# mlrun/mlrun

Hardware: NVIDIA H100
Metric: events/sec (higher is better)
Workload: dtype f32 in / f64 accumulate

## Files before the change

mlrun_b200/csrc/b2s_rowthread.cuh:

```cuda
#pragma once
#include <cuda.h>
#include <type_traits>

#include "b2s_device.cuh"
#include "b2s_hash.cuh"

namespace b2s {

constexpr int kRTMaxCatCols = 16;
constexpr int kRTCatsInline = 4;
constexpr int kRTMaxCats = 256;

template <int NCH, int NS>
struct RTParams {
  const char* rows;
  int64_t row_stride;
  int64_t n_rows;
  float* out;
  int32_t* status;
  int32_t n_in, out_cols, n_models, vote_kind, out_is_int, fast_epilogue, tile_rows, pitch, stages, vec_ok;
  int32_t n_cat_cols, n_cat;
  int32_t one_sync;
  int32_t use_bulk;
  float* peers[8];
  int64_t peer_off;
  int32_t n_peers;
  MergeSig sig;
  const double* wcat;
  const double* vote_w_g;
  const ModelDesc* models;
  const int32_t* classes;
  double w[NCH * 4][NS];
  float fill[NCH * 4];
  float lim[NCH * 4];
  double bias[NS];
  double vote_w[NS];
  int32_t cat_col[kRTMaxCatCols];
  int32_t cat_off[kRTMaxCatCols];
  int32_t cat_sw[kRTMaxCatCols];
  int32_t cat_base[kRTMaxCatCols];
  int32_t cat_cnt[kRTMaxCatCols];
  float cat_fill[kRTMaxCatCols];
  float cat_inl[kRTMaxCatCols][kRTCatsInline];
  int32_t cat_first[kRTMaxCatCols];
  int32_t cat_dense[kRTMaxCatCols];
  float cat_val[kRTMaxCats];
  struct CatFast {
    int32_t off_b;
    int32_t sw_b;
    int32_t first;
    int32_t cnt;
    int32_t woff_b;
    float fill;
    int32_t pad[2];
  };
  CatFast catf[kRTMaxCatCols];
  int32_t cats_fast;
  int32_t zero_woff_b;
  int32_t dead_tail;
  int32_t pad_fast;
  const long long* g_keys;
  const TableSlot* g_slots;
  uint64_t g_mask;
  const float* g_values;
  long long g_missing_row;
};

struct RowPadded {
  const float* xr;
  __device__ __forceinline__ float4 chunk(int ch) const { return *reinterpret_cast<const float4*>(xr + ch * 4); }
  __device__ __forceinline__ float at2(int off, int) const { return xr[off]; }
  __device__ __forceinline__ float at_b(int off_b, int) const { return *reinterpret_cast<const float*>(reinterpret_cast<const char*>(xr) + off_b); }
};
struct RowSwizzled {
  const float* box0;
  int box_words;
  int r7s;
  __device__ __forceinline__ float4 chunk(int ch) const {
    return *reinterpret_cast<const float4*>(box0 + (ch >> 3) * box_words + (((ch & 7) << 2) ^ r7s));
  }
  __device__ __forceinline__ float at2(int off, int sw) const { return box0[off + (sw ^ r7s)]; }
  __device__ __forceinline__ float at_b(int off_b, int sw_b) const {
    return *reinterpret_cast<const float*>(reinterpret_cast<const char*>(box0) + off_b + (sw_b ^ (r7s << 2)));
  }
};

template <int NCH, int NS, int CH0, int CH1, typename Row>
__device__ __forceinline__ void rt_slice(const RTParams<NCH, NS>& p, const Row (&xr)[1], double (&acc)[1][NS]) {
  constexpr int RPT = 1;
  constexpr int BATCH = 4;
#pragma unroll
  for (int b = CH0; b < CH1; b += BATCH) {
    double xd[RPT][BATCH * 4];
#pragma unroll
    for (int cb = 0; cb < BATCH; ++cb) {
      const int ch = b + cb;
      if (ch < CH1) {
#pragma unroll
        for (int i = 0; i < RPT; ++i) {
          const float4 v = xr[i].chunk(ch);
          const float xs[4] = {v.x, v.y, v.z, v.w};
#pragma unroll
          for (int u = 0; u < 4; ++u) {
            const int c = ch * 4 + u;
            float x = xs[u];
            x = !(fabsf(x) <= p.lim[c]) ? p.fill[c] : x;
            xd[i][cb * 4 + u] = (double)x;
          }
        }
      }
    }
#pragma unroll
    for (int cb = 0; cb < BATCH; ++cb) {
      const int ch = b + cb;
      if (ch < CH1) {
#pragma unroll
        for (int u = 0; u < 4; ++u) {
          const int c = ch * 4 + u;
#pragma unroll
          for (int k = 0; k < NS; ++k)
#pragma unroll
            for (int i = 0; i < RPT; ++i) acc[i][k] = fma(p.w[c][k], xd[i][cb * 4 + u], acc[i][k]);
        }
      }
    }
  }
}

template <int NCH, int NS>
__device__ __noinline__ int rt_cat_search(const RTParams<NCH, NS>& p, int cc, float x) {
  const int b0 = p.cat_base[cc], cnt = p.cat_cnt[cc];
  int j = p.n_cat;
  if (cnt <= kRTCatsInline) {
#pragma unroll
    for (int qq = kRTCatsInline - 1; qq >= 0; --qq) j = (x == p.cat_inl[cc][qq]) ? b0 + qq : j;
  } else {
    for (int qq = cnt - 1; qq >= 0; --qq) j = (x == p.cat_val[b0 + qq]) ? b0 + qq : j;
  }
  return j;
}

template <int NCH, int NS, int Q0, int TPR, typename Row>
__device__ __forceinline__ void rt_cats(const RTParams<NCH, NS>& p, const Row (&xr)[1], const double* __restrict__ s_wcat,
                                        double (&acc)[1][NS]) {
  constexpr int RPT = 1;
  constexpr int ITERS = (kRTMaxCatCols - Q0 + TPR - 1) / TPR;
  if (p.cats_fast) {
    const char* wb = reinterpret_cast<const char*>(s_wcat);
#pragma unroll
    for (int it = 0; it < ITERS; ++it) {
      const int cc = Q0 + it * TPR;
      if (cc >= p.n_cat_cols) break;
      const typename RTParams<NCH, NS>::CatFast cf = p.catf[cc];
#pragma unroll
      for (int i = 0; i < RPT; ++i) {
        float x = xr[i].at_b(cf.off_b, cf.sw_b);
        x = (x != x) ? cf.fill : x;
        const int v = __float2int_rz(x);
        const unsigned jj = (unsigned)(v - cf.first);
        const bool miss = ((float)v != x) | (jj >= (unsigned)cf.cnt);
        const int a = miss ? p.zero_woff_b : cf.woff_b + (int)jj * (NS * 8);
        if constexpr (NS % 2 == 0) {
#pragma unroll
          for (int k = 0; k < NS; k += 2) {
            const double2 w2 = *reinterpret_cast<const double2*>(wb + a + k * 8);
            acc[i][k] += w2.x;
            acc[i][k + 1] += w2.y;
          }
        } else {
          const double* wc = reinterpret_cast<const double*>(wb + a);
#pragma unroll
          for (int k = 0; k < NS; ++k) acc[i][k] += wc[k];
        }
      }
    }
    return;
  }
#pragma unroll
  for (int it = 0; it < ITERS; ++it) {
    const int cc = Q0 + it * TPR;
    if (cc >= p.n_cat_cols) break;
#pragma unroll
    for (int i = 0; i < RPT; ++i) {
      float x = xr[i].at2(p.cat_off[cc], p.cat_sw[cc]);
      x = (x != x) ? p.cat_fill[cc] : x;
      int j;
      if (p.cat_dense[cc]) {
        const int v = __float2int_rz(x);
        const unsigned jj = (unsigned)(v - p.cat_first[cc]);
        j = ((float)v == x && jj < (unsigned)p.cat_cnt[cc]) ? p.cat_base[cc] + (int)jj : p.n_cat;
      } else {
        j = rt_cat_search(p, cc, x);
      }
      const double* wc = s_wcat + (size_t)j * NS;
#pragma unroll
      for (int k = 0; k < NS; ++k) acc[i][k] += wc[k];
    }
  }
}

template <int NCH, int NS, int TPR, int LIVE, typename Row>
__device__ __forceinline__ void rt_row_slices(const RTParams<NCH, NS>& p, int q, const Row (&xr)[1], const double* __restrict__ s_wcat,
                                              double (&acc)[1][NS]) {
  static_assert(LIVE % TPR == 0, "live chunks must split evenly over the row's threads");
  constexpr int CPT = LIVE / TPR;
  if (TPR == 1 || q == 0) {
    rt_slice<NCH, NS, 0, CPT>(p, xr, acc);
    rt_cats<NCH, NS, 0, TPR>(p, xr, s_wcat, acc);
  } else if (q == 1) {
    rt_slice<NCH, NS, (TPR > 1 ? CPT : 0), (TPR > 1 ? 2 * CPT : 0)>(p, xr, acc);
    rt_cats<NCH, NS, (TPR > 1 ? 1 : 0), TPR>(p, xr, s_wcat, acc);
  } else if (q == 2) {
    rt_slice<NCH, NS, (TPR > 2 ? 2 * CPT : 0), (TPR > 2 ? 3 * CPT : 0)>(p, xr, acc);
    rt_cats<NCH, NS, (TPR > 2 ? 2 : 0), TPR>(p, xr, s_wcat, acc);
  } else {
    rt_slice<NCH, NS, (TPR > 3 ? 3 * CPT : 0), (TPR > 3 ? 4 * CPT : 0)>(p, xr, acc);
    rt_cats<NCH, NS, (TPR > 3 ? 3 : 0), TPR>(p, xr, s_wcat, acc);
  }
}

__device__ __forceinline__ void mbar_init(uint64_t* bar, int count) {
  asm volatile("mbarrier.init.shared::cta.b64 [%0], %1;" ::"r"((uint32_t)__cvta_generic_to_shared(bar)), "r"(count));
}
__device__ __forceinline__ void mbar_expect_tx(uint64_t* bar, uint32_t bytes) {
  asm volatile("mbarrier.arrive.expect_tx.shared::cta.b64 _, [%0], %1;" ::"r"((uint32_t)__cvta_generic_to_shared(bar)), "r"(bytes)
               : "memory");
}
__device__ __forceinline__ void mbar_wait(uint64_t* bar, uint32_t parity) {
  const uint32_t a = (uint32_t)__cvta_generic_to_shared(bar);
  asm volatile(
      "{\n"
      ".reg .pred p;\n"
      "WAIT_%=:\n"
      "mbarrier.try_wait.parity.shared::cta.b64 p, [%0], %1;\n"
      "@p bra DONE_%=;\n"
      "bra WAIT_%=;\n"
      "DONE_%=:\n"
      "}\n" ::"r"(a), "r"(parity)
      : "memory");
}
__device__ __forceinline__ void bulk_load(void* smem_dst, const void* gsrc, uint32_t bytes, uint64_t* bar) {
  asm volatile("cp.async.bulk.shared::cluster.global.mbarrier::complete_tx::bytes [%0], [%1], %2, [%3];" ::"r"(
                   (uint32_t)__cvta_generic_to_shared(smem_dst)),
               "l"(gsrc), "r"(bytes), "r"((uint32_t)__cvta_generic_to_shared(bar))
               : "memory");
}

__device__ __forceinline__ void tensor_load_2d(void* smem_dst, const CUtensorMap* tmap, int x, int y, uint64_t* bar) {
  asm volatile(
      "cp.async.bulk.tensor.2d.shared::cluster.global.tile.mbarrier::complete_tx::bytes [%0], [%1, {%2, %3}], [%4];" ::"r"(
          (uint32_t)__cvta_generic_to_shared(smem_dst)),
// ... 1 lines not shown
      : "memory");
}

template <int NCH, int NS>
__device__ __noinline__ void rt_generic_epilogue(const RTParams<NCH, NS>& p, const double* sl, int64_t row, uint32_t st) {
  double pred[kMaxModels];
  for (int m = 0; m < p.n_models; ++m) {
    const ModelDesc md = p.models[m];
    pred[m] = apply_link(md, sl + md.score_off, p.classes);
  }
  KParams kp;
  kp.out = p.out;
  kp.out_cols = p.out_cols;
  kp.n_models = p.n_models;
  kp.vote_kind = p.vote_kind;
  kp.out_is_int = p.out_is_int;
  kp.vote_w = p.vote_w_g;
  kp.status = p.status;
  kp.n_peers = p.n_peers;
  kp.peer_off = p.peer_off;
  for (int g = 0; g < p.n_peers; ++g) kp.peers[g] = p.peers[g];
  vote_and_store(kp, pred, row, st);
}

template <int NCH, int NS, int TPR, int LM>
__global__ void __launch_bounds__(128 * TPR, TPR >= 4 ? 2 : (TPR == 2 ? 3 : 4))
    rowthread_kernel(const __grid_constant__ RTParams<NCH, NS> p, const __grid_constant__ CUtensorMap tmap) {
  constexpr int RPT = 1;
  static_assert(NCH % TPR == 0, "chunks must split evenly over the row's threads");
  constexpr int CPT = NCH / TPR;
  extern __shared__ __align__(16) unsigned char smem[];
  uint64_t* s_bar = reinterpret_cast<uint64_t*>(smem);
  double* s_wcat = reinterpret_cast<double*>(smem + 64);
  const size_t wcat_bytes = 64 + (((size_t)(p.n_cat + 1) * NS * 8 + 15) / 16) * 16;
  const bool one_sync = (LM == 2) && TPR > 1 && p.one_sync;
  constexpr size_t part_words = (size_t)(TPR - 1) * 128 * NS;
  double* s_part = reinterpret_cast<double*>(smem + wcat_bytes);
  float* s_tiles = reinterpret_cast<float*>(smem + wcat_bytes + (one_sync ? 2 : 1) * part_words * 8);
  if (LM == 2) {
    const uint32_t a = (uint32_t)__cvta_generic_to_shared(s_tiles);
    s_tiles += ((1024u - (a & 1023u)) & 1023u) >> 2;
  }

  const int tid = threadIdx.x;
  const int TR = p.tile_rows;
  const int S = p.stages;
  const int tile_words = (LM == 2) ? TR * NCH * 4 : TR * p.pitch;
  const int64_t n_tiles = (p.n_rows + TR - 1) / TR;
  const int TRT = TR / RPT;
  const int q = tid / TRT;
  const int r = tid - q * TRT;

  const int cprv = p.vec_ok ? (p.n_in >> 2) : p.n_in;
  const int r0 = tid / cprv, c0 = tid - r0 * cprv;
  const int dr = (int)blockDim.x / cprv, dc = (int)blockDim.x - dr * cprv;
  auto issue = [&](float* tile, int64_t row0) {
    int64_t left = p.n_rows - row0;
    const int rows = left < TR ? (left < 0 ? 0 : (int)left) : TR;
    const char* base = p.rows + row0 * p.row_stride;
    int rr = r0, cc = c0;
    if (p.vec_ok) {
      while (rr < rows) {
        cp_async16(tile + rr * p.pitch + cc * 4, base + (int64_t)rr * p.row_stride + cc * 16);
        rr += dr;
        cc += dc;
        if (cc >= cprv) {
          cc -= cprv;
          ++rr;
// ... 66 lines not shown
            unknown_bits = (unknown_bits & ~(1u << st)) | ((hit < 0 ? 1u : 0u) << st);
            bulk_load(s_tiles + st * tile_words + tid * p.pitch,
                      reinterpret_cast<const char*>(p.g_values + (hit < 0 ? p.g_missing_row : hit) * p.n_in), row_bytes, &s_bar[st]);
          }
          gk_cur = gk_nxt;
          g_probe_start(gk_cur);
          gk_nxt = g_key(g_tile_nxt);
          g_tile_nxt += gridDim.x;
        }
      } else if (tid < rows) {
        bulk_load(s_tiles + st * tile_words + tid * p.pitch, p.rows + (row0 + tid) * p.row_stride, row_bytes, &s_bar[st]);
      }
    }
  };
  if (bulk) {
    if (tid == 0) {
      for (int s = 0; s < S; ++s) mbar_init(&s_bar[s], 1);
      asm volatile("fence.mbarrier_init.release.cluster;" ::: "memory");
    }
    __syncthreads();
  }
  for (int s = 0; s < (one_sync ? S : S - 1); ++s) {
    const int64_t t = (int64_t)blockIdx.x + (int64_t)s * gridDim.x;
    if (bulk) {
      issue_bulk(s, t * TR);
    } else {
      if (t < n_tiles) issue(s_tiles + s * tile_words, t * TR);
      cp_async_commit();
    }
  }
  uint32_t phase_bits = 0;
  for (int i = tid; i < p.n_cat * NS; i += blockDim.x) s_wcat[i] = p.wcat[i];
  for (int i = tid; i < NS; i += blockDim.x) s_wcat[p.n_cat * NS + i] = 0.0;
  if (one_sync) __syncthreads();

  int stage = 0;
  uint32_t iter = 0;
  for (int64_t t = blockIdx.x; t < n_tiles; t += gridDim.x) {
    if (bulk) {
      mbar_wait(&s_bar[stage], (phase_bits >> stage) & 1u);
      phase_bits ^= (1u << stage);
    } else if (S == 2) cp_async_wait<0>();
    else if (S == 3) cp_async_wait<1>();
    else cp_async_wait<2>();
    if (!one_sync) {
      __syncthreads();
      const int64_t tn = t + (int64_t)(S - 1) * gridDim.x;
      int sn = stage + S - 1;
      if (sn >= S) sn -= S;
      if (bulk) {
        issue_bulk(sn, tn * TR);
      } else {
        if (tn < n_tiles) issue(s_tiles + sn * tile_words, tn * TR);
        cp_async_commit();
      }
    }
    const float* tile = s_tiles + stage * tile_words;
    const int64_t row0 = t * TR;
    const int live_rows = (int)(p.n_rows - row0 < (int64_t)TR ? p.n_rows - row0 : (int64_t)TR);
    const bool any_live = r < live_rows;
    using Row = typename std::conditional<LM == 2, RowSwizzled, RowPadded>::type;
    Row xr[RPT];
#pragma unroll
    for (int i = 0; i < RPT; ++i) {
      const int ri = r + i * TRT;
      if constexpr (LM == 2) {
        xr[i].box0 = tile + ri * 32;
        xr[i].box_words = TR * 32;
        xr[i].r7s = (r & 7) << 2;
      } else {
        xr[i].xr = tile + ri * p.pitch;
      }
    }
    double acc[RPT][NS];
#pragma unroll
    for (int i = 0; i < RPT; ++i)
#pragma unroll
      for (int k = 0; k < NS; ++k) acc[i][k] = 0.0;
    if (any_live) {
      if constexpr (LM == 2 && RPT == 1 && NCH >= 8 && (TPR == 1 || TPR == 2)) {
        if (p.dead_tail >= 4) rt_row_slices<NCH, NS, TPR, NCH - 4>(p, q, xr, s_wcat, acc);
        else if (p.dead_tail >= 2) rt_row_slices<NCH, NS, TPR, NCH - 2>(p, q, xr, s_wcat, acc);
        else rt_row_slices<NCH, NS, TPR, NCH>(p, q, xr, s_wcat, acc);
      } else {
        rt_row_slices<NCH, NS, TPR, NCH>(p, q, xr, s_wcat, acc);
      }
    }
    if (TPR > 1) {
      double* s_part_cur = s_part + (one_sync ? (size_t)(iter & 1) * part_words : 0);
      if (q > 0) {
#pragma unroll
        for (int i = 0; i < RPT; ++i) {
          double* part = s_part_cur + ((size_t)(q - 1) * 128 + r + i * TRT) * NS;
#pragma unroll
          for (int k = 0; k < NS; ++k) part[k] = acc[i][k];
        }
      }
      __syncthreads();
      if (one_sync) issue_bulk(stage, (t + (int64_t)S * gridDim.x) * TR);
      if (q == 0) {
#pragma unroll
        for (int i = 0; i < RPT; ++i)
#pragma unroll
          for (int qq = 1; qq < TPR; ++qq) {
            const double* o = s_part_cur + ((size_t)(qq - 1) * 128 + r + i * TRT) * NS;
#pragma unroll
            for (int k = 0; k < NS; ++k) acc[i][k] += o[k];
          }
      }
    }
#pragma unroll
    for (int i = 0; i < RPT; ++i) {
      const int64_t row = row0 + (r + i * TRT);
      if (q == 0 && r + i * TRT < live_rows) {
        uint32_t st = 0;
#pragma unroll
        for (int k = 0; k < NS; ++k) {
          acc[i][k] += p.bias[k];
          st |= (fabs(acc[i][k]) <= 1.7976931348623157e308) ? 0u : 1u;
        }
        if (LM == 1) st |= ((unknown_bits >> stage) & 1u) << 2;
        if (p.fast_epilogue) {
          if (p.vote_kind == 1) {
            double s = 0.0;
#pragma unroll
            for (int k = 0; k < NS; ++k) s = __dadd_rn(s, __dmul_rn(acc[i][k], p.vote_w[k]));
            store_word(p, row, 0, __float_as_uint((float)s));
          } else {
#pragma unroll
            for (int k = 0; k < NS; ++k)
              if (k < p.n_models) store_word(p, row, k, __float_as_uint((float)acc[i][k]));
          }
          if (p.status) p.status[row] = (int32_t)st;
        } else {
          double sl[NS];
#pragma unroll
          for (int k = 0; k < NS; ++k) sl[k] = acc[i][k];
          rt_generic_epilogue(p, sl, row, st);
        }
      }
    }
    ++stage;
    ++iter;
    if (stage == S) stage = 0;
  }
  cp_async_wait<0>();
  merge_signal(p.sig);
}

}
```

mlrun_b200/csrc/b2s_runtime.cu:

```cuda
#include <cuda_runtime.h>

#include <exception>

#include <algorithm>
#include <atomic>
#include <chrono>
#include <cmath>
#include <condition_variable>
#include <cstdarg>
#include <cstdio>
#include <cstdlib>
#include <cstring>
#include <deque>
#include <limits>
#include <map>
#include <memory>
#include <mutex>
#include <string>
#include <thread>
#include <vector>

#include "../../include/b200serve.h"
#include "b2s_internal.h"
#include "b2s_device.cuh"
// ... 128 lines not shown
  int fused_lag = -1;
  uint32_t fused_epoch = 0;
  size_t bytes = 0;
  bool connected = false;
  size_t buf_bytes() const { return (size_t)world * max_rows * out_cols * 4; }
  char* buf(int r, uint32_t e) const { return peer_base[r] + kCommHeader + (size_t)(e & (kCommSlots - 1u)) * buf_bytes(); }
  uint32_t* flags(int r) const { return reinterpret_cast<uint32_t*>(peer_base[r]); }
  uint32_t* counter() const { return reinterpret_cast<uint32_t*>(base.get()) + 64; }
  uint32_t* timeout_flag() const { return reinterpret_cast<uint32_t*>(base.get()) + 65; }
};

struct b2s_plan_s {
  int32_t n_in = 0;
  bool finalized = false;
  std::vector<float> fill;
  std::vector<std::vector<MapEntry>> maps;
  std::vector<int32_t> out_src, out_kind;
  std::vector<float> out_arg;
  std::vector<HostModel> models;
  int vote_kind = B2S_VOTE_NONE;
  std::vector<double> vote_w;
  int mode = MODE_STORE;
  int NS = 1;
  int out_cols = 0;
  int out_is_int = 0;
  KParams kp{};
  DeviceArray<char> d_blob;
  size_t blob_bytes = 0;
  int grid = 0, block = 0;
  int kernels_per_batch = 1;
  bool rt_ok = false;
  int rt_cat_cols = 0;
  int rt_NCH = 0, rt_NS = 0, rt_grid = 0, rt_smem = 0, rt_pitch = 0;
  std::vector<char> rt_blob;
  std::vector<void*> peers;
  int64_t peer_off = 0;
  struct b2s_comm_s* comm = nullptr;
  bool dense_ok = false;
  DenseParams dense{};
  int dense_smem = 0, dense_grid = 0;
  std::atomic<int32_t> last_kernel{B2S_KERNEL_NONE};
  bool t3_ok = false, t3_miss = false, t3_cat = false;
  bool any_cat = false;
  int t3_D = 0, t3_grid = 0, t3_block = 0, t3_smem = 0, t3_cols = 0, t3_parts = 0;
  T3Params t3{};
  T3Prep t3_prep{};
  int t3_prep_smem = 0;
  DeviceArray<char> d_t3_blob;
  const int32_t* d_t3_col_score = nullptr;
  const int32_t* d_t3_col_order = nullptr;
  const int32_t* d_t3_model_cols = nullptr;
  struct TreeScratch {
    DeviceArray<double> partial;
    DeviceArray<int32_t> row_bad;
    DeviceArray<uint32_t> xt;
    int64_t rows = 0;
    std::mutex mu;
    int reserve(int64_t n, int cols, int xt_words) {
      if (n <= rows) return B2S_OK;
      rows = 0;
      const int64_t cap = std::max<int64_t>((n + 63) / 64 * 64, 65536);
      if (int rc = allocate(partial, (size_t)cap * cols * 8)) return rc;
      if (int rc = allocate(row_bad, (size_t)cap * 4)) return rc;
      if (int rc = allocate(xt, (size_t)(cap / kT3TR) * xt_words * 4)) return rc;
      rows = cap;
      return B2S_OK;
// ... 82 lines not shown
    if (cudaGetDriverEntryPoint("cuTensorMapEncodeTiled", &sym, cudaEnableDefault, &q) != cudaSuccess || q != cudaDriverEntryPointSuccess) {
      cudaGetLastError();
      sym = nullptr;
    }
    return reinterpret_cast<EncodeTiledFn>(sym);
  }();
  return fn;
}
static bool encode_rows_map(CUtensorMap* map, const void* rows, int64_t n_rows, int64_t stride, int n_in, int tile_rows) {
  EncodeTiledFn enc = tensor_map_encoder();
  if (!enc) return false;
  cuuint64_t gdim[2] = {(cuuint64_t)n_in, (cuuint64_t)n_rows};
  cuuint64_t gstride[1] = {(cuuint64_t)stride};
  cuuint32_t box[2] = {32u, (cuuint32_t)tile_rows};
  cuuint32_t estr[2] = {1u, 1u};
  return enc(map, CU_TENSOR_MAP_DATA_TYPE_FLOAT32, 2, const_cast<void*>(rows), gdim, gstride, box, estr,
             CU_TENSOR_MAP_INTERLEAVE_NONE, CU_TENSOR_MAP_SWIZZLE_128B, CU_TENSOR_MAP_L2_PROMOTION_L2_128B,
             CU_TENSOR_MAP_FLOAT_OOB_FILL_NONE) == CUDA_SUCCESS;
}

struct RTTables {
  int n_in, n_out_cols, n_models, vote_kind, out_is_int, fast_epilogue, NS;
  const std::vector<float>* fill;
  const std::vector<uint32_t>* flags;
  const std::vector<double>* wnum;
  const std::vector<double>* bias;
  const std::vector<double>* vote_w;
  const std::vector<int32_t>* cat_off;
  const std::vector<float>* cat_val;
  const double* d_wcat;
  const double* d_vote_w;
  const ModelDesc* d_models;
  const int32_t* d_classes;
};

constexpr int rt_tpr(int NCH) { return NCH >= 8 ? 2 : 1; }
constexpr int kRTTileRows = 128, kRTStages = 2;

template <int NCH, int NS>
static void rt_build(b2s_plan_s* p, const RTTables& t) {
  using P = RTParams<NCH, NS>;
  p->rt_blob.assign(sizeof(P), 0);
  P& r = *reinterpret_cast<P*>(p->rt_blob.data());
  r.n_in = t.n_in;
  r.out_cols = t.n_out_cols;
  r.n_models = t.n_models;
  r.vote_kind = t.vote_kind;
  r.out_is_int = t.out_is_int;
  r.fast_epilogue = t.fast_epilogue;
  r.wcat = t.d_wcat;
  r.vote_w_g = t.d_vote_w;
  r.models = t.d_models;
  r.classes = t.d_classes;
  for (int c = 0; c < NCH * 4; ++c) {
    r.fill[c] = 0.0f;
    r.lim[c] = -1.0f;
    for (int k = 0; k < NS; ++k) r.w[c][k] = 0.0;
  }
  for (int c = 0; c < t.n_in; ++c) {
    const bool input = ((*t.flags)[c] & COL_COPIED) != 0;
    r.fill[c] = input ? (*t.fill)[c] : 0.0f;
    r.lim[c] = input ? std::numeric_limits<float>::infinity() : -1.0f;
    for (int k = 0; k < NS; ++k) r.w[c][k] = (*t.wnum)[(size_t)c * NS + k];
  }
  for (int k = 0; k < NS; ++k) {
    r.bias[k] = k < (int)t.bias->size() ? (*t.bias)[k] : 0.0;
    r.vote_w[k] = k < (int)t.vote_w->size() ? (*t.vote_w)[k] : 0.0;
// ... 5 lines not shown
      r.cat_base[ncc] = (*t.cat_off)[c];
      r.cat_cnt[ncc] = (*t.cat_off)[c + 1] - (*t.cat_off)[c];
      r.cat_fill[ncc] = (*t.fill)[c];
      for (int q = 0; q < kRTCatsInline; ++q)
        r.cat_inl[ncc][q] = q < r.cat_cnt[ncc] ? (*t.cat_val)[r.cat_base[ncc] + q] : std::numeric_limits<float>::quiet_NaN();
      {
        const float f0 = (*t.cat_val)[r.cat_base[ncc]];
        bool dense = f0 == std::floor(f0) && std::fabs(f0) < 8388608.0f;
        for (int q = 0; dense && q < r.cat_cnt[ncc]; ++q) dense = (*t.cat_val)[r.cat_base[ncc] + q] == f0 + (float)q;
        r.cat_dense[ncc] = dense ? 1 : 0;
        r.cat_first[ncc] = dense ? (int)f0 : 0;
      }
      ++ncc;
    }
  r.n_cat_cols = ncc;
  r.n_cat = (int)t.cat_val->size();
  r.cats_fast = 1;
  for (int cc = 0; cc < ncc; ++cc) {
    r.cats_fast = r.cats_fast && r.cat_dense[cc];
    r.catf[cc].first = r.cat_first[cc];
    r.catf[cc].cnt = r.cat_cnt[cc];
    r.catf[cc].woff_b = r.cat_base[cc] * NS * 8;
    r.catf[cc].fill = r.cat_fill[cc];
  }
  r.zero_woff_b = r.n_cat * NS * 8;
  {
    int last_live = -1;
    for (int c = 0; c < t.n_in; ++c)
      if (((*t.flags)[c] & COL_COPIED) != 0) last_live = c >> 2;
    r.dead_tail = std::max(0, NCH - 1 - last_live);
    if (last_live < 0) r.dead_tail = 0;
  }
  for (int i = 0; i < r.n_cat; ++i) r.cat_val[i] = (*t.cat_val)[i];
}

struct LaunchCtx {
  const KParams* k = nullptr;
  bool host_rows = false;
};

template <int NCH, int NS>
static cudaError_t rt_launch_t(b2s_plan_s* p, const void* rows, int64_t stride, int64_t n_rows, void* out, int32_t* status,
                               int vec_ok, cudaStream_t st, bool query, int* occ, const B2SGather* gather, const LaunchCtx* lc) {
  using P = RTParams<NCH, NS>;
  constexpr int TPR = rt_tpr(NCH);
  constexpr int LMT = NCH >= 8 ? 2 : 1;
  static std::atomic<bool> attr_set{false};
  if (!attr_set) {
    const int cap = (int)G.prop.sharedMemPerBlockOptin;
    cudaError_t e = cudaFuncSetAttribute(rowthread_kernel<NCH, NS, TPR, 0>, cudaFuncAttributeMaxDynamicSharedMemorySize, cap);
    if (e == cudaSuccess) e = cudaFuncSetAttribute(rowthread_kernel<NCH, NS, TPR, 1>, cudaFuncAttributeMaxDynamicSharedMemorySize, cap);
    if (e == cudaSuccess && NCH >= 8)
      e = cudaFuncSetAttribute(rowthread_kernel<NCH, NS, TPR, LMT>, cudaFuncAttributeMaxDynamicSharedMemorySize, cap);
    if (e != cudaSuccess) return e;
    attr_set = true;
  }
  const bool tmap_ok = NCH >= 8 && p->n_in == NCH * 4 && tensor_map_encoder() != nullptr;
  if (query) {
    if (tmap_ok)
      return cudaOccupancyMaxActiveBlocksPerMultiprocessor(occ, rowthread_kernel<NCH, NS, TPR, LMT>, kRTTileRows * TPR, p->rt_smem);
    return cudaOccupancyMaxActiveBlocksPerMultiprocessor(occ, rowthread_kernel<NCH, NS, TPR, 0>, kRTTileRows * TPR, p->rt_smem);
  }
  P r = *reinterpret_cast<const P*>(p->rt_blob.data());
  r.rows = (const char*)rows;
  r.row_stride = stride;
  r.n_rows = n_rows;
// ... 924 lines not shown
    {
      const char* denv = getenv("B2S_DENSE");
      int n_cat_cols = 0;
      for (int c = 0; c < n_in; ++c) n_cat_cols += (cat_off[c + 1] > cat_off[c]) ? 1 : 0;
      bool all_copied = true;
      for (int c = 0; c < n_in; ++c) all_copied = all_copied && (flags[c] & COL_COPIED);
      if ((!denv || atoi(denv) != 0) && p->mode == MODE_LINEAR && total_scores > 8 && total_scores <= 32 && identity_schema &&
          !any_map && n_cat_cols == 0 && all_copied && (n_in % 32) == 0 && n_in <= kDenseMaxIn) {
        dense_pad = total_scores <= 16 ? 16 : 32;
        dense_wh.assign((size_t)dense_pad * n_in, 0.0f);
        dense_wm.assign((size_t)dense_pad * n_in, 0.0f);
        dense_wl.assign((size_t)dense_pad * n_in, 0.0f);
        auto tf32 = [](double x) {
          float f = (float)x;
          if (!std::isfinite(f)) return f;
          uint32_t b;
          memcpy(&b, &f, 4);
          b &= 0xffffe000u;
          memcpy(&f, &b, 4);
          return f;
        };
        for (int kk = 0; kk < total_scores; ++kk)
          for (int c = 0; c < n_in; ++c) {
            const double w = wnum[(size_t)c * NS + kk];
            const float hi = tf32(w);
            const double r1 = w - (double)hi;
            const float mid = tf32(r1);
            dense_wh[(size_t)kk * n_in + c] = hi;
            dense_wm[(size_t)kk * n_in + c] = mid;
            dense_wl[(size_t)kk * n_in + c] = tf32(r1 - (double)mid);
          }
      }
    }
    BlobBuilder bb;
    const size_t o_dwh = bb.add(dense_wh), o_dwm = bb.add(dense_wm), o_dwl = bb.add(dense_wl);
    const size_t o_fill = bb.add(p->fill), o_flags = bb.add(flags), o_mapoff = bb.add(map_off), o_maps = bb.add(maps),
                 o_osrc = bb.add(p->out_src), o_okind = bb.add(p->out_kind), o_oarg = bb.add(p->out_arg),
                 o_catoff = bb.add(cat_off), o_catval = bb.add(cat_val), o_wnum = bb.add(wnum), o_wcat = bb.add(wcat),
                 o_bias = bb.add(bias), o_models = bb.add(descs), o_classes = bb.add(classes),
                 o_votew = bb.add(p->vote_w), o_wgen = bb.add(wgen), o_nodes = bb.add(nodes), o_leaf = bb.add(leaf),
                 o_troot = bb.add(tree_root), o_tslot = bb.add(tree_slot), o_tscale = bb.add(tree_scale),
                 o_chunk = bb.add(chunk_kind);
    B2S_CUDA_TRY(cudaSetDevice(G.device));
    if (int rc = allocate(p->d_blob, bb.data.size())) return rc;
    B2S_CUDA_TRY(cudaMemcpy(p->d_blob.get(), bb.data.data(), bb.data.size(), cudaMemcpyHostToDevice));
    p->blob_bytes = bb.data.size();
    char* B = p->d_blob.get();

    KParams& k = p->kp;
    memset(&k, 0, sizeof(k));
    k.n_in = n_in;
    k.n_out = n_out;
    k.out_cols = p->out_cols;
    k.n_models = M;
    k.n_scores = total_scores;
    k.vote_kind = p->vote_kind;
    k.out_is_int = p->out_is_int;
    k.need_expand = need_expand ? 1 : 0;
    k.models_pow2 = pow2_at_least(std::max(M, 1));
    k.n_cat = (int)cat_val.size();
    k.n_maps = (int)maps.size();
    k.fill = (const float*)(B + o_fill);
    k.col_flags = (const uint32_t*)(B + o_flags);
    k.map_off = (const int32_t*)(B + o_mapoff);
    k.maps = (const MapEntry*)(B + o_maps);
    k.out_src = (const int32_t*)(B + o_osrc);
    k.out_kind = (const int32_t*)(B + o_okind);
    k.out_arg = (const float*)(B + o_oarg);
    k.cat_off = (const int32_t*)(B + o_catoff);
    k.cat_val = (const float*)(B + o_catval);
    k.wnum = (const double*)(B + o_wnum);
    k.wcat = (const double*)(B + o_wcat);
    k.bias = (const double*)(B + o_bias);
    k.models = (const ModelDesc*)(B + o_models);
    k.classes = (const int32_t*)(B + o_classes);
    k.vote_w = (const double*)(B + o_votew);
    k.wgen = (const double*)(B + o_wgen);
    k.nodes = (const TreeNode*)(B + o_nodes);
    k.leaf = (const double*)(B + o_leaf);
    k.tree_root = (const int32_t*)(B + o_troot);
    k.tree_slot = (const int32_t*)(B + o_tslot);
    k.tree_scale = (const double*)(B + o_tscale);
    k.chunk_kind = (const uint8_t*)(B + o_chunk);
    if (dense_pad > 0 && tensor_map_encoder() != nullptr) {
      DenseParams& d = p->dense;
      memset(&d, 0, sizeof(d));
      d.wh = (const float*)(B + o_dwh);
      d.wm = (const float*)(B + o_dwm);
      d.wl = (const float*)(B + o_dwl);
      d.fill = k.fill;
      d.bias = k.bias;
      d.n_in = n_in;
      d.n_scores = total_scores;
      d.n_pad = dense_pad;
      d.exact = (getenv("B2S_DENSE_EXACT") && atoi(getenv("B2S_DENSE_EXACT")) != 0) ? 1 : 0;
      d.any_fill = any_fill ? 1 : 0;
      for (int kk = 0; kk < 32; ++kk) {
        d.biasf[kk] = kk < total_scores ? (float)bias[kk] : 0.0f;
        d.votewf[kk] = 0.0f;
        d.labels[kk] = kk;
      }
      {
        bool simple = true;
        for (auto& m : p->models) simple = simple && m.link == B2S_LINK_IDENTITY && m.n_scores == 1;
        d.epi = DENSE_EPI_GENERIC;
        if (simple && p->vote_kind == B2S_VOTE_NONE) d.epi = DENSE_EPI_SCORES;
        if (simple && p->vote_kind == B2S_VOTE_MEAN) {
          d.epi = DENSE_EPI_MEAN;
          for (int mi = 0; mi < M; ++mi) d.votewf[mi] = (float)p->vote_w[mi];
        }
        if (M == 1 && p->models[0].link == B2S_LINK_ARGMAX && p->vote_kind == B2S_VOTE_NONE) {
          d.epi = DENSE_EPI_ARGMAX;
          const auto& cls = p->models[0].classes;
          for (int kk = 0; kk < total_scores && kk < 32; ++kk) d.labels[kk] = cls.empty() ? kk : cls[kk];
        }
      }
      p->dense_smem = dense_smem_bytes(n_in, dense_pad);
      if (p->dense_smem <= (int)G.prop.sharedMemPerBlockOptin) {
        p->dense_grid = G.prop.multiProcessorCount;
        p->dense_ok = true;
      }
    }

    const int n_in4 = (int)align_up(n_in, 4);
    int pitch = n_in4 + 4;
    if (((pitch / 4) & 1) == 0) pitch += 4;
    int exp_pitch = n_out | 1;
    const int smem_cap = (int)G.prop.sharedMemPerBlockOptin;
    const int sms = G.prop.multiProcessorCount;
    int block, tile_rows, stages, blocks_per_sm;
    int tpr = 1;
    if (p->mode == MODE_LINEAR) {
      tpr = NS <= 8 ? 4 : (NS == 16 ? 2 : 1);
      const int nch = (n_in + 3) / 4;
      while (tpr > 1 && nch < tpr * 2) tpr /= 2;
      tile_rows = 128;
      block = tile_rows * tpr;
// ... 46 lines not shown
      total = carve(tile_rows, stages);
    }
    if (total > smem_cap) {
      if (p->mode == MODE_LINEAR) {
        while (total > smem_cap && tile_rows > 8) {
          tile_rows /= 2;
          total = carve(tile_rows, stages);
        }
      }
      if (total > smem_cap) return fail(B2S_ERR_UNSUPPORTED, "plan needs %d B shared memory > %d B", total, smem_cap);
    }
    if (p->mode == MODE_TREES) block = std::max(32, tile_rows * k.models_pow2);
    if (p->mode == MODE_LINEAR) block = tile_rows * tpr;
    k.tpr = tpr;
    k.sm_total = total;
    k.tile_rows = tile_rows;
    k.pitch = pitch;
    k.exp_pitch = exp_pitch;
    k.stages = stages;
    p->NS = NS;
    p->block = block;
    int occ = std::max(1, std::min(blocks_per_sm, smem_cap / std::max(total, 1)));
    p->grid = sms * occ;

    {
      int n_cat_cols = 0;
      for (int c = 0; c < n_in; ++c) n_cat_cols += (cat_off[c + 1] > cat_off[c]) ? 1 : 0;
      if (p->mode == MODE_LINEAR && !any_map && n_in <= 128 && NS <= 8 && n_cat_cols <= kRTMaxCatCols &&
          (int)cat_val.size() <= kRTMaxCats) {
        const int nch = (n_in + 3) / 4;
        p->rt_NCH = nch <= 4 ? 4 : (nch <= 8 ? 8 : (nch <= 16 ? 16 : 32));
        p->rt_NS = NS;
        p->rt_cat_cols = n_cat_cols;
        bool simple = true;
        for (auto& m : p->models) simple = simple && m.link == B2S_LINK_IDENTITY && m.n_scores == 1;
        RTTables t{n_in, p->out_cols, M, p->vote_kind, p->out_is_int, (simple && p->vote_kind != B2S_VOTE_MAJORITY) ? 1 : 0, NS,
                   &p->fill, &flags, &wnum, &bias, &p->vote_w, &cat_off, &cat_val, k.wcat, k.vote_w, k.models, k.classes};
        rt_build_any(p, t);
        int rpitch = p->rt_NCH * 4 + 4;
        if (((rpitch / 4) & 1) == 0) rpitch += 4;
        p->rt_pitch = rpitch;
        {
          const size_t fixed = 1024 + 64 + align_up((size_t)(cat_val.size() + 1) * NS * 8, 16);
          const size_t part = (size_t)(rt_tpr(p->rt_NCH) - 1) * 128 * NS * 8;
          const size_t padded = fixed + part + (size_t)kRTStages * kRTTileRows * rpitch * 4;
          const size_t swizzled = fixed + 2 * part + (size_t)kRTStages * kRTTileRows * p->rt_NCH * 16;
          p->rt_smem = (int)std::max(padded, swizzled);
        }
        int occ = 0;
        if (p->rt_smem <= smem_cap && rt_launch(p, nullptr, 0, 0, nullptr, nullptr, 0, nullptr, true, &occ) == cudaSuccess && occ >= 1) {
          p->rt_ok = true;
          p->rt_grid = sms * occ;
        } else {
          cudaGetLastError();
        }
      }
    }
    if (p->mode == MODE_TREES && identity_schema && !any_map) {
      if (int rc = t3_build(p, k, any_fill)) return rc;
    }
    if (int rc = p->ev.create(2)) return rc;
    p->finalized = true;
    return B2S_OK;
  } catch (const std::exception& e) {
    return fail(B2S_ERR_INVALID, "%s: %s", __func__, e.what());
  }
}

extern "C" const char* b2s_plan_kernel(b2s_plan_t p) {
  if (!p || !p->finalized) return "";
  static thread_local char buf[200];
  const bool tmap = p->rt_NCH >= 8 && p->n_in == p->rt_NCH * 4 && tensor_map_encoder();
  if (p->dense_ok) snprintf(buf, sizeof(buf), "dense_head_kernel<N=%d> (wgmma tf32, %s, register accumulator groups; %d scores over %d columns)", p->dense.n_pad, p->dense.exact ? "exact 3-term input split" : "2-term input split", p->dense.n_scores, p->dense.n_in);
  else if (p->t3_ok) snprintf(buf, sizeof(buf), "t3_prep_kernel + trees3_kernel<D=%d,%s%s> + t3_vote_kernel (%d parts resident in shared memory, %d walking warps)", p->t3_D, p->t3_miss ? "NaN routing" : "floats", p->t3_cat ? ",categorical" : "", p->t3_parts, p->t3.warps);
  else if (p->rt_ok) snprintf(buf, sizeof(buf), "rowthread_kernel<NCH=%d,NS=%d,TPR=%d,%s>", p->rt_NCH, p->rt_NS, rt_tpr(p->rt_NCH), tmap ? "TMA tensor-map loads" : "TMA bulk loads");
  else snprintf(buf, sizeof(buf), "rows_kernel<%s,NS=%d>%s", p->mode == MODE_LINEAR ? "LINEAR" : (p->mode == MODE_TREES ? "TREES" : "STORE"), p->NS, p->any_cat ? " (categorical splits)" : "");
  return buf;
}

extern "C" int32_t b2s_plan_last_kernel(b2s_plan_t p) {
  return p ? p->last_kernel.load(std::memory_order_relaxed) : B2S_KERNEL_NONE;
}

extern "C" int b2s_plan_out_info(b2s_plan_t p, int32_t* out_cols, int32_t* out_is_int) {
  try {
    if (!p || !p->finalized) return fail(B2S_ERR_STATE, "plan not finalized");
    if (out_cols) *out_cols = p->out_cols;
    if (out_is_int) *out_is_int = p->out_is_int;
    return B2S_OK;
  } catch (const std::exception& e) {
    return fail(B2S_ERR_INVALID, "%s: %s", __func__, e.what());
  }
}

struct NvtxRange {
  explicit NvtxRange(const char* name) { nvtxRangePushA(name); }
  ~NvtxRange() { nvtxRangePop(); }
};

static int launch_on(b2s_plan_t p, const void* d_rows, int64_t n_rows, int64_t stride, void* d_out, int32_t* d_status,
                     cudaStream_t st, bool host_rows = false) {
  if (n_rows == 0 && !p->comm) return B2S_OK;
  NvtxRange nvtx(p->dense_ok ? "b2s:dense_head" : p->t3_ok ? "b2s:trees3 (prep+walk+vote)"
                 : p->rt_ok ? "b2s:rowthread" : p->mode == MODE_STORE ? "b2s:rows_store" : "b2s:rows_kernel");
  KParams k = p->kp;
  k.rows = (const char*)d_rows;
  k.row_stride = stride;
  k.n_rows = n_rows;
// ... 922 lines not shown
```

Baseline: 10.56 billion.

## Fold mean-vote linear ensemble into a single weight vector on host

When all linear models use identity links with one score each and are combined by a weighted mean vote, the per-model weights, categorical weights and biases are pre-combined on the host with compensated summation into a single model. The row-thread kernel then accumulates one double per row instead of NS, which cuts FMAs, shared-memory partial traffic and register pressure. Rows whose folded sum overflows fall back to an exact unfolded recomputation. The trade-offs are a slightly different rounding order, extra shared memory for the folded categorical table, and the one-sync double-buffer path being turned off when folding is on.

Measured after the change: 11.05 billion, median of 6. +4.6%, better.

```diff
diff --git a/mlrun_b200/csrc/b2s_rowthread.cuh b/mlrun_b200/csrc/b2s_rowthread.cuh
--- a/mlrun_b200/csrc/b2s_rowthread.cuh
+++ b/mlrun_b200/csrc/b2s_rowthread.cuh
@@ -52,7 +52,8 @@
     int32_t cnt;
     int32_t woff_b;
     float fill;
-    int32_t pad[2];
+    int32_t woff_fb;
+    int32_t pad;
   };
   CatFast catf[kRTMaxCatCols];
   int32_t cats_fast;
@@ -64,6 +65,11 @@
   uint64_t g_mask;
   const float* g_values;
   long long g_missing_row;
+  int32_t folded;
+  int32_t zero_woff_fb;
+  const double* wcat_f;
+  double bias_f;
+  double wf[NCH * 4];
 };
 
 struct RowPadded {
@@ -85,8 +91,10 @@
   }
 };
 
-template <int NCH, int NS, int CH0, int CH1, typename Row>
-__device__ __forceinline__ void rt_slice(const RTParams<NCH, NS>& p, const Row (&xr)[1], double (&acc)[1][NS]) {
+template <int NCH, int NS, int NA, int CH0, int CH1, typename Row>
+__device__ __forceinline__ void rt_slice(const RTParams<NCH, NS>& p, const Row (&xr)[1], double (&acc)[1][NA]) {
+  static_assert(NA == NS || NA == 1, "score slots or the folded model");
+  constexpr bool F = NA != NS;
   constexpr int RPT = 1;
   constexpr int BATCH = 4;
 #pragma unroll
@@ -118,9 +126,9 @@
         for (int u = 0; u < 4; ++u) {
           const int c = ch * 4 + u;
 #pragma unroll
-          for (int k = 0; k < NS; ++k)
-#pragma unroll
-            for (int i = 0; i < RPT; ++i) acc[i][k] = fma(p.w[c][k], xd[i][cb * 4 + u], acc[i][k]);
+          for (int k = 0; k < NA; ++k)
+#pragma unroll
+            for (int i = 0; i < RPT; ++i) acc[i][k] = fma(F ? p.wf[c] : p.w[c][k], xd[i][cb * 4 + u], acc[i][k]);
         }
       }
     }
@@ -140,11 +148,12 @@
   return j;
 }
 
-template <int NCH, int NS, int Q0, int TPR, typename Row>
+template <int NCH, int NS, int NA, int Q0, int TPR, typename Row>
 __device__ __forceinline__ void rt_cats(const RTParams<NCH, NS>& p, const Row (&xr)[1], const double* __restrict__ s_wcat,
-                                        double (&acc)[1][NS]) {
+                                        double (&acc)[1][NA]) {
   constexpr int RPT = 1;
   constexpr int ITERS = (kRTMaxCatCols - Q0 + TPR - 1) / TPR;
+  constexpr bool F = NA != NS;
   if (p.cats_fast) {
     const char* wb = reinterpret_cast<const char*>(s_wcat);
 #pragma unroll
@@ -159,10 +168,10 @@
         const int v = __float2int_rz(x);
         const unsigned jj = (unsigned)(v - cf.first);
         const bool miss = ((float)v != x) | (jj >= (unsigned)cf.cnt);
-        const int a = miss ? p.zero_woff_b : cf.woff_b + (int)jj * (NS * 8);
-        if constexpr (NS % 2 == 0) {
-#pragma unroll
-          for (int k = 0; k < NS; k += 2) {
+        const int a = miss ? (F ? p.zero_woff_fb : p.zero_woff_b) : (F ? cf.woff_fb : cf.woff_b) + (int)jj * (NA * 8);
+        if constexpr (NA % 2 == 0) {
+#pragma unroll
+          for (int k = 0; k < NA; k += 2) {
             const double2 w2 = *reinterpret_cast<const double2*>(wb + a + k * 8);
             acc[i][k] += w2.x;
             acc[i][k + 1] += w2.y;
@@ -170,7 +179,7 @@
         } else {
           const double* wc = reinterpret_cast<const double*>(wb + a);
 #pragma unroll
-          for (int k = 0; k < NS; ++k) acc[i][k] += wc[k];
+          for (int k = 0; k < NA; ++k) acc[i][k] += wc[k];
         }
       }
     }
@@ -192,31 +201,63 @@
       } else {
         j = rt_cat_search(p, cc, x);
       }
-      const double* wc = s_wcat + (size_t)j * NS;
-#pragma unroll
-      for (int k = 0; k < NS; ++k) acc[i][k] += wc[k];
-    }
-  }
-}
-
-template <int NCH, int NS, int TPR, int LIVE, typename Row>
+      const double* wc = s_wcat + (size_t)j * NA;
+#pragma unroll
+      for (int k = 0; k < NA; ++k) acc[i][k] += wc[k];
+    }
+  }
+}
+
+template <int NCH, int NS, int NA, int TPR, int LIVE, typename Row>
 __device__ __forceinline__ void rt_row_slices(const RTParams<NCH, NS>& p, int q, const Row (&xr)[1], const double* __restrict__ s_wcat,
-                                              double (&acc)[1][NS]) {
+                                              double (&acc)[1][NA]) {
   static_assert(LIVE % TPR == 0, "live chunks must split evenly over the row's threads");
   constexpr int CPT = LIVE / TPR;
   if (TPR == 1 || q == 0) {
-    rt_slice<NCH, NS, 0, CPT>(p, xr, acc);
-    rt_cats<NCH, NS, 0, TPR>(p, xr, s_wcat, acc);
+    rt_slice<NCH, NS, NA, 0, CPT>(p, xr, acc);
+    rt_cats<NCH, NS, NA, 0, TPR>(p, xr, s_wcat, acc);
   } else if (q == 1) {
-    rt_slice<NCH, NS, (TPR > 1 ? CPT : 0), (TPR > 1 ? 2 * CPT : 0)>(p, xr, acc);
-    rt_cats<NCH, NS, (TPR > 1 ? 1 : 0), TPR>(p, xr, s_wcat, acc);
+    rt_slice<NCH, NS, NA, (TPR > 1 ? CPT : 0), (TPR > 1 ? 2 * CPT : 0)>(p, xr, acc);
+    rt_cats<NCH, NS, NA, (TPR > 1 ? 1 : 0), TPR>(p, xr, s_wcat, acc);
   } else if (q == 2) {
-    rt_slice<NCH, NS, (TPR > 2 ? 2 * CPT : 0), (TPR > 2 ? 3 * CPT : 0)>(p, xr, acc);
-    rt_cats<NCH, NS, (TPR > 2 ? 2 : 0), TPR>(p, xr, s_wcat, acc);
+    rt_slice<NCH, NS, NA, (TPR > 2 ? 2 * CPT : 0), (TPR > 2 ? 3 * CPT : 0)>(p, xr, acc);
+    rt_cats<NCH, NS, NA, (TPR > 2 ? 2 : 0), TPR>(p, xr, s_wcat, acc);
   } else {
-    rt_slice<NCH, NS, (TPR > 3 ? 3 * CPT : 0), (TPR > 3 ? 4 * CPT : 0)>(p, xr, acc);
-    rt_cats<NCH, NS, (TPR > 3 ? 3 : 0), TPR>(p, xr, s_wcat, acc);
-  }
+    rt_slice<NCH, NS, NA, (TPR > 3 ? 3 * CPT : 0), (TPR > 3 ? 4 * CPT : 0)>(p, xr, acc);
+    rt_cats<NCH, NS, NA, (TPR > 3 ? 3 : 0), TPR>(p, xr, s_wcat, acc);
+  }
+}
+
+template <int NCH, int NS, typename Row>
+__device__ __forceinline__ double rt_unfolded_vote(const RTParams<NCH, NS>& p, const Row& row, const double* __restrict__ s_wcat) {
+  double acc[NS];
+#pragma unroll
+  for (int k = 0; k < NS; ++k) acc[k] = 0.0;
+#pragma unroll 1
+  for (int ch = 0; ch < NCH; ++ch) {
+    const float4 v = row.chunk(ch);
+    const float xs[4] = {v.x, v.y, v.z, v.w};
+#pragma unroll
+    for (int u = 0; u < 4; ++u) {
+      const int c = ch * 4 + u;
+      const float x = !(fabsf(xs[u]) <= p.lim[c]) ? p.fill[c] : xs[u];
+#pragma unroll
+      for (int k = 0; k < NS; ++k) acc[k] = fma(p.w[c][k], (double)x, acc[k]);
+    }
+  }
+#pragma unroll 1
+  for (int cc = 0; cc < p.n_cat_cols; ++cc) {
+    float x = row.at2(p.cat_off[cc], p.cat_sw[cc]);
+    x = (x != x) ? p.cat_fill[cc] : x;
+    int j = p.n_cat;
+    for (int qq = p.cat_cnt[cc] - 1; qq >= 0; --qq) j = (x == p.cat_val[p.cat_base[cc] + qq]) ? p.cat_base[cc] + qq : j;
+#pragma unroll
+    for (int k = 0; k < NS; ++k) acc[k] += s_wcat[(size_t)j * NS + k];
+  }
+  double s = 0.0;
+#pragma unroll
+  for (int k = 0; k < NS; ++k) s = __dadd_rn(s, __dmul_rn(__dadd_rn(acc[k], p.bias[k]), p.vote_w[k]));
+  return s;
 }
 
 __device__ __forceinline__ void mbar_init(uint64_t* bar, int count) {
@@ -284,8 +325,11 @@
   extern __shared__ __align__(16) unsigned char smem[];
   uint64_t* s_bar = reinterpret_cast<uint64_t*>(smem);
   double* s_wcat = reinterpret_cast<double*>(smem + 64);
-  const size_t wcat_bytes = 64 + (((size_t)(p.n_cat + 1) * NS * 8 + 15) / 16) * 16;
-  const bool one_sync = (LM == 2) && TPR > 1 && p.one_sync;
+  const bool fold = NS >= 2 && p.folded;
+  const size_t wcat_model_bytes = (((size_t)(p.n_cat + 1) * NS * 8 + 15) / 16) * 16;
+  double* s_wcatf = reinterpret_cast<double*>(smem + 64 + wcat_model_bytes);
+  const size_t wcat_bytes = 64 + wcat_model_bytes + (fold ? (((size_t)(p.n_cat + 1) * 8 + 15) / 16) * 16 : 0);
+  const bool one_sync = (LM == 2) && TPR > 1 && p.one_sync && !fold;
   constexpr size_t part_words = (size_t)(TPR - 1) * 128 * NS;
   double* s_part = reinterpret_cast<double*>(smem + wcat_bytes);
   float* s_tiles = reinterpret_cast<float*>(smem + wcat_bytes + (one_sync ? 2 : 1) * part_words * 8);
@@ -418,6 +462,8 @@
   uint32_t phase_bits = 0;
   for (int i = tid; i < p.n_cat * NS; i += blockDim.x) s_wcat[i] = p.wcat[i];
   for (int i = tid; i < NS; i += blockDim.x) s_wcat[p.n_cat * NS + i] = 0.0;
+  if (fold)
+    for (int i = tid; i <= p.n_cat; i += blockDim.x) s_wcatf[i] = i < p.n_cat ? p.wcat_f[i] : 0.0;
   if (one_sync) __syncthreads();
 
   int stage = 0;
@@ -458,74 +504,85 @@
         xr[i].xr = tile + ri * p.pitch;
       }
     }
-    double acc[RPT][NS];
-#pragma unroll
-    for (int i = 0; i < RPT; ++i)
-#pragma unroll
-      for (int k = 0; k < NS; ++k) acc[i][k] = 0.0;
-    if (any_live) {
-      if constexpr (LM == 2 && RPT == 1 && NCH >= 8 && (TPR == 1 || TPR == 2)) {
-        if (p.dead_tail >= 4) rt_row_slices<NCH, NS, TPR, NCH - 4>(p, q, xr, s_wcat, acc);
-        else if (p.dead_tail >= 2) rt_row_slices<NCH, NS, TPR, NCH - 2>(p, q, xr, s_wcat, acc);
-        else rt_row_slices<NCH, NS, TPR, NCH>(p, q, xr, s_wcat, acc);
-      } else {
-        rt_row_slices<NCH, NS, TPR, NCH>(p, q, xr, s_wcat, acc);
-      }
-    }
-    if (TPR > 1) {
-      double* s_part_cur = s_part + (one_sync ? (size_t)(iter & 1) * part_words : 0);
-      if (q > 0) {
-#pragma unroll
-        for (int i = 0; i < RPT; ++i) {
-          double* part = s_part_cur + ((size_t)(q - 1) * 128 + r + i * TRT) * NS;
-#pragma unroll
-          for (int k = 0; k < NS; ++k) part[k] = acc[i][k];
-        }
-      }
-      __syncthreads();
-      if (one_sync) issue_bulk(stage, (t + (int64_t)S * gridDim.x) * TR);
-      if (q == 0) {
-#pragma unroll
-        for (int i = 0; i < RPT; ++i)
-#pragma unroll
-          for (int qq = 1; qq < TPR; ++qq) {
-            const double* o = s_part_cur + ((size_t)(qq - 1) * 128 + r + i * TRT) * NS;
-#pragma unroll
-            for (int k = 0; k < NS; ++k) acc[i][k] += o[k];
+    auto score_tile = [&](auto na) {
+      constexpr int NA = decltype(na)::value;
+      constexpr bool F = NA != NS;
+      const double* s_w = F ? s_wcatf : s_wcat;
+      double acc[RPT][NA];
+#pragma unroll
+      for (int i = 0; i < RPT; ++i)
+#pragma unroll
+        for (int k = 0; k < NA; ++k) acc[i][k] = 0.0;
+      if (any_live) {
+        if constexpr (LM == 2 && RPT == 1 && NCH >= 8 && (TPR == 1 || TPR == 2)) {
+          if (p.dead_tail >= 4) rt_row_slices<NCH, NS, NA, TPR, NCH - 4>(p, q, xr, s_w, acc);
+          else if (p.dead_tail >= 2) rt_row_slices<NCH, NS, NA, TPR, NCH - 2>(p, q, xr, s_w, acc);
+          else rt_row_slices<NCH, NS, NA, TPR, NCH>(p, q, xr, s_w, acc);
+        } else {
+          rt_row_slices<NCH, NS, NA, TPR, NCH>(p, q, xr, s_w, acc);
+        }
+      }
+      if (TPR > 1) {
+        double* s_part_cur = s_part + (one_sync ? (size_t)(iter & 1) * part_words : 0);
+        if (q > 0) {
+#pragma unroll
+          for (int i = 0; i < RPT; ++i) {
+            double* part = s_part_cur + ((size_t)(q - 1) * 128 + r + i * TRT) * NA;
+#pragma unroll
+            for (int k = 0; k < NA; ++k) part[k] = acc[i][k];
           }
-      }
-    }
-#pragma unroll
-    for (int i = 0; i < RPT; ++i) {
-      const int64_t row = row0 + (r + i * TRT);
-      if (q == 0 && r + i * TRT < live_rows) {
-        uint32_t st = 0;
-#pragma unroll
-        for (int k = 0; k < NS; ++k) {
-          acc[i][k] += p.bias[k];
-          st |= (fabs(acc[i][k]) <= 1.7976931348623157e308) ? 0u : 1u;
-        }
-        if (LM == 1) st |= ((unknown_bits >> stage) & 1u) << 2;
-        if (p.fast_epilogue) {
-          if (p.vote_kind == 1) {
-            double s = 0.0;
-#pragma unroll
-            for (int k = 0; k < NS; ++k) s = __dadd_rn(s, __dmul_rn(acc[i][k], p.vote_w[k]));
+        }
+        __syncthreads();
+        if (one_sync) issue_bulk(stage, (t + (int64_t)S * gridDim.x) * TR);
+        if (q == 0) {
+#pragma unroll
+          for (int i = 0; i < RPT; ++i)
+#pragma unroll
+            for (int qq = 1; qq < TPR; ++qq) {
+              const double* o = s_part_cur + ((size_t)(qq - 1) * 128 + r + i * TRT) * NA;
+#pragma unroll
+              for (int k = 0; k < NA; ++k) acc[i][k] += o[k];
+            }
+        }
+      }
+#pragma unroll
+      for (int i = 0; i < RPT; ++i) {
+        const int64_t row = row0 + (r + i * TRT);
+        if (q == 0 && r + i * TRT < live_rows) {
+          uint32_t st = 0;
+#pragma unroll
+          for (int k = 0; k < NA; ++k) {
+            acc[i][k] += F ? p.bias_f : p.bias[k];
+            st |= (fabs(acc[i][k]) <= 1.7976931348623157e308) ? 0u : 1u;
+          }
+          if (LM == 1) st |= ((unknown_bits >> stage) & 1u) << 2;
+          if constexpr (F) {
+            const double s = (st & 1u) ? rt_unfolded_vote<NCH, NS>(p, xr[i], s_wcat) : acc[i][0];
             store_word(p, row, 0, __float_as_uint((float)s));
+            if (p.status) p.status[row] = (int32_t)st;
+          } else if (p.fast_epilogue) {
+            if (p.vote_kind == 1) {
+              double s = 0.0;
+#pragma unroll
+              for (int k = 0; k < NS; ++k) s = __dadd_rn(s, __dmul_rn(acc[i][k], p.vote_w[k]));
+              store_word(p, row, 0, __float_as_uint((float)s));
+            } else {
+#pragma unroll
+              for (int k = 0; k < NS; ++k)
+                if (k < p.n_models) store_word(p, row, k, __float_as_uint((float)acc[i][k]));
+            }
+            if (p.status) p.status[row] = (int32_t)st;
           } else {
-#pragma unroll
-            for (int k = 0; k < NS; ++k)
-              if (k < p.n_models) store_word(p, row, k, __float_as_uint((float)acc[i][k]));
+            double sl[NS];
+#pragma unroll
+            for (int k = 0; k < NS; ++k) sl[k] = acc[i][k];
+            rt_generic_epilogue(p, sl, row, st);
           }
-          if (p.status) p.status[row] = (int32_t)st;
-        } else {
-          double sl[NS];
-#pragma unroll
-          for (int k = 0; k < NS; ++k) sl[k] = acc[i][k];
-          rt_generic_epilogue(p, sl, row, st);
-        }
-      }
-    }
+        }
+      }
+    };
+    if (NS >= 2 && fold) score_tile(std::integral_constant<int, 1>{});
+    else score_tile(std::integral_constant<int, NS>{});
     ++stage;
     ++iter;
     if (stage == S) stage = 0;
diff --git a/mlrun_b200/csrc/b2s_runtime.cu b/mlrun_b200/csrc/b2s_runtime.cu
--- a/mlrun_b200/csrc/b2s_runtime.cu
+++ b/mlrun_b200/csrc/b2s_runtime.cu
@@ -184,6 +184,7 @@
   bool rt_ok = false;
   int rt_cat_cols = 0;
   int rt_NCH = 0, rt_NS = 0, rt_grid = 0, rt_smem = 0, rt_pitch = 0;
+  bool rt_folded = false;
   std::vector<char> rt_blob;
   std::vector<void*> peers;
   int64_t peer_off = 0;
@@ -332,7 +333,37 @@
   const double* d_vote_w;
   const ModelDesc* d_models;
   const int32_t* d_classes;
+  const std::vector<double>* wnum_f;
+  double bias_f;
+  const double* d_wcat_f;
 };
+
+static bool fold_mean_vote(int NS, const std::vector<double>& vote_w, const std::vector<double>& wnum,
+                           const std::vector<double>& wcat, const std::vector<double>& bias, std::vector<double>& wnum_f,
+                           std::vector<double>& wcat_f, double& bias_f) {
+  constexpr double kBound = 0x1p880;
+  const int M = (int)vote_w.size();
+  auto fold = [&](const double* w, double& out) {
+    double hi = 0.0, lo = 0.0, mag = 0.0;
+    for (int k = 0; k < M; ++k) {
+      if (!(std::fabs(w[k]) < kBound)) return false;
+      const double pr = vote_w[k] * w[k], pe = std::fma(vote_w[k], w[k], -pr);
+      const double sum = hi + pr, bv = sum - hi, se = (hi - (sum - bv)) + (pr - bv);
+      hi = sum;
+      lo += se + pe;
+      mag += std::fabs(pr);
+    }
+    out = hi + lo;
+    return mag < kBound;
+  };
+  wnum_f.assign(wnum.size() / NS, 0.0);
+  wcat_f.assign(wcat.size() / NS, 0.0);
+  for (size_t c = 0; c < wnum_f.size(); ++c)
+    if (!fold(&wnum[c * NS], wnum_f[c])) return false;
+  for (size_t j = 0; j < wcat_f.size(); ++j)
+    if (!fold(&wcat[j * NS], wcat_f[j])) return false;
+  return fold(bias.data(), bias_f);
+}
 
 constexpr int rt_tpr(int NCH) { return NCH >= 8 ? 2 : 1; }
 constexpr int kRTTileRows = 128, kRTStages = 2;
@@ -404,6 +435,15 @@
     if (last_live < 0) r.dead_tail = 0;
   }
   for (int i = 0; i < r.n_cat; ++i) r.cat_val[i] = (*t.cat_val)[i];
+  p->rt_folded = NS >= 2 && t.wnum_f != nullptr;
+  if (p->rt_folded) {
+    r.folded = 1;
+    for (int c = 0; c < t.n_in; ++c) r.wf[c] = (*t.wnum_f)[c];
+    r.bias_f = t.bias_f;
+    r.wcat_f = t.d_wcat_f;
+    for (int cc = 0; cc < ncc; ++cc) r.catf[cc].woff_fb = r.cat_base[cc] * 8;
+    r.zero_woff_fb = r.n_cat * 8;
+  }
 }
 
 struct LaunchCtx {
@@ -1394,6 +1434,12 @@
           }
       }
     }
+    bool simple = true;
+    for (auto& m : p->models) simple = simple && m.link == B2S_LINK_IDENTITY && m.n_scores == 1;
+    std::vector<double> wnum_f, wcat_f;
+    double bias_f = 0.0;
+    const bool folded = p->mode == MODE_LINEAR && p->vote_kind == B2S_VOTE_MEAN && simple && NS >= 2 &&
+                        fold_mean_vote(NS, p->vote_w, wnum, wcat, bias, wnum_f, wcat_f, bias_f);
     BlobBuilder bb;
     const size_t o_dwh = bb.add(dense_wh), o_dwm = bb.add(dense_wm), o_dwl = bb.add(dense_wl);
     const size_t o_fill = bb.add(p->fill), o_flags = bb.add(flags), o_mapoff = bb.add(map_off), o_maps = bb.add(maps),
@@ -1402,7 +1448,7 @@
                  o_bias = bb.add(bias), o_models = bb.add(descs), o_classes = bb.add(classes),
                  o_votew = bb.add(p->vote_w), o_wgen = bb.add(wgen), o_nodes = bb.add(nodes), o_leaf = bb.add(leaf),
                  o_troot = bb.add(tree_root), o_tslot = bb.add(tree_slot), o_tscale = bb.add(tree_scale),
-                 o_chunk = bb.add(chunk_kind);
+                 o_chunk = bb.add(chunk_kind), o_wcatf = bb.add(wcat_f);
     B2S_CUDA_TRY(cudaSetDevice(G.device));
     if (int rc = allocate(p->d_blob, bb.data.size())) return rc;
     B2S_CUDA_TRY(cudaMemcpy(p->d_blob.get(), bb.data.data(), bb.data.size(), cudaMemcpyHostToDevice));
@@ -1463,8 +1509,6 @@
         d.labels[kk] = kk;
       }
       {
-        bool simple = true;
-        for (auto& m : p->models) simple = simple && m.link == B2S_LINK_IDENTITY && m.n_scores == 1;
         d.epi = DENSE_EPI_GENERIC;
         if (simple && p->vote_kind == B2S_VOTE_NONE) d.epi = DENSE_EPI_SCORES;
         if (simple && p->vote_kind == B2S_VOTE_MEAN) {
@@ -1577,19 +1621,19 @@
         p->rt_NCH = nch <= 4 ? 4 : (nch <= 8 ? 8 : (nch <= 16 ? 16 : 32));
         p->rt_NS = NS;
         p->rt_cat_cols = n_cat_cols;
-        bool simple = true;
-        for (auto& m : p->models) simple = simple && m.link == B2S_LINK_IDENTITY && m.n_scores == 1;
         RTTables t{n_in, p->out_cols, M, p->vote_kind, p->out_is_int, (simple && p->vote_kind != B2S_VOTE_MAJORITY) ? 1 : 0, NS,
-                   &p->fill, &flags, &wnum, &bias, &p->vote_w, &cat_off, &cat_val, k.wcat, k.vote_w, k.models, k.classes};
+                   &p->fill, &flags, &wnum, &bias, &p->vote_w, &cat_off, &cat_val, k.wcat, k.vote_w, k.models, k.classes,
+                   folded ? &wnum_f : nullptr, bias_f, (const double*)(B + o_wcatf)};
         rt_build_any(p, t);
         int rpitch = p->rt_NCH * 4 + 4;
         if (((rpitch / 4) & 1) == 0) rpitch += 4;
         p->rt_pitch = rpitch;
         {
-          const size_t fixed = 1024 + 64 + align_up((size_t)(cat_val.size() + 1) * NS * 8, 16);
+          const size_t fixed = 1024 + 64 + align_up((size_t)(cat_val.size() + 1) * NS * 8, 16) +
+                               (p->rt_folded ? align_up((size_t)(cat_val.size() + 1) * 8, 16) : 0);
           const size_t part = (size_t)(rt_tpr(p->rt_NCH) - 1) * 128 * NS * 8;
           const size_t padded = fixed + part + (size_t)kRTStages * kRTTileRows * rpitch * 4;
-          const size_t swizzled = fixed + 2 * part + (size_t)kRTStages * kRTTileRows * p->rt_NCH * 16;
+          const size_t swizzled = fixed + (p->rt_folded ? 1 : 2) * part + (size_t)kRTStages * kRTTileRows * p->rt_NCH * 16;
           p->rt_smem = (int)std::max(padded, swizzled);
         }
         int occ = 0;
@@ -1618,7 +1662,7 @@
   const bool tmap = p->rt_NCH >= 8 && p->n_in == p->rt_NCH * 4 && tensor_map_encoder();
   if (p->dense_ok) snprintf(buf, sizeof(buf), "dense_head_kernel<N=%d> (wgmma tf32, %s, register accumulator groups; %d scores over %d columns)", p->dense.n_pad, p->dense.exact ? "exact 3-term input split" : "2-term input split", p->dense.n_scores, p->dense.n_in);
   else if (p->t3_ok) snprintf(buf, sizeof(buf), "t3_prep_kernel + trees3_kernel<D=%d,%s%s> + t3_vote_kernel (%d parts resident in shared memory, %d walking warps)", p->t3_D, p->t3_miss ? "NaN routing" : "floats", p->t3_cat ? ",categorical" : "", p->t3_parts, p->t3.warps);
-  else if (p->rt_ok) snprintf(buf, sizeof(buf), "rowthread_kernel<NCH=%d,NS=%d,TPR=%d,%s>", p->rt_NCH, p->rt_NS, rt_tpr(p->rt_NCH), tmap ? "TMA tensor-map loads" : "TMA bulk loads");
+  else if (p->rt_ok) snprintf(buf, sizeof(buf), "rowthread_kernel<NCH=%d,NS=%d,TPR=%d,%s>%s", p->rt_NCH, p->rt_NS, rt_tpr(p->rt_NCH), tmap ? "TMA tensor-map loads" : "TMA bulk loads", p->rt_folded ? ", mean vote folded" : "");
   else snprintf(buf, sizeof(buf), "rows_kernel<%s,NS=%d>%s", p->mode == MODE_LINEAR ? "LINEAR" : (p->mode == MODE_TREES ? "TREES" : "STORE"), p->NS, p->any_cat ? " (categorical splits)" : "");
   return buf;
 }
```
